# RiceChuan/teku

Measured on AMD Instinct MI355X. Metric: BLS sigs verified/sec (batchVerify), 1-8 GPUs; p50 latency @128-sig batch, higher is better.
Workload: dtype u32 (381-bit Montgomery Fp, 14x29-bit limb products); 1 GPU; config 5 per-GPU shard: randomized batchVerify of 131072 single-signer sets per GPU, RCCL Fp12 partial gather, 1 final exp; sets_per_gpu=131072, parallelism=data-parallel shards, dp1

## Files before the change

__graft_entry__.py:

```python

import os
import subprocess
import sys

ROOT = os.path.dirname(os.path.abspath(__file__))
CSRC = os.path.join(ROOT, "teku_amd", "csrc")
LIBDIR = os.path.join(ROOT, "teku_amd", "lib")
HIPCC = os.environ.get("HIPCC", "/opt/rocm/bin/hipcc")
ARCH = "gfx950"


def _run(cmd):
    print("+", " ".join(cmd), flush=True)
    subprocess.check_call(cmd, cwd=ROOT)


def _stale(out, deps):
    if not os.path.exists(out):
        return True
    t = os.path.getmtime(out)
    return any(os.path.getmtime(d) > t for d in deps)


def _includes(path, seen=None):
    import re

    seen = set() if seen is None else seen
    path = os.path.normpath(path)
    if path in seen or not os.path.exists(path):
        return seen
    seen.add(path)
    for m in re.finditer(r'^\s*#\s*include\s+"([^"]+)"', open(path).read(), re.M):
        _includes(os.path.join(os.path.dirname(path), m.group(1)), seen)
    return seen


def _csrc_deps():
    return [os.path.join(CSRC, f) for f in os.listdir(CSRC) if f.endswith((".h", ".hip"))] + [
        os.path.join(ROOT, "include", "tekubls.h")
    ]


HIP_TUS = ["tb_lib.hip", "tb_kzg.hip", "k_keys.hip", "k_pkindex.hip", "k_sigs.hip", "k_hash.hip", "k_mwave.hip", "k_hwave.hip", "k_hrow.hip", "k_kcoop.hip", "k_lines.hip", "k_pair.hip", "k_each.hip", "k_kzg.hip", "k_w2_hash.hip", "k_w2_sig.hip", "k_w2_pk.hip", "k_hquad.hip", "k_w2_lines.hip", "tb_hostdec.hip"]


def build_hip_lib(force=False, jobs=None, variant=None, defines=(), only=None):
    from concurrent.futures import ThreadPoolExecutor

    os.makedirs(LIBDIR, exist_ok=True)
    objdir = os.path.join(LIBDIR, "obj" if not variant else f"obj_{variant}")
    os.makedirs(objdir, exist_ok=True)
    if variant:
        os.makedirs(os.path.join(LIBDIR, "variants"), exist_ok=True)
    out = os.path.join(LIBDIR, "libtekubls_hip.so" if not variant else os.path.join("variants", f"libtekubls_hip_{variant}.so"))
    deps = _csrc_deps()
    flags = [f"--offload-arch={ARCH}", "-O3", "-std=c++17", "-fPIC"] + [f"-D{d}" for d in defines]

    def compile_tu(tu):
        if variant and only and tu not in only:
            return os.path.join(LIBDIR, "obj", tu.replace(".hip", ".o"))
        obj = os.path.join(objdir, tu.replace(".hip", ".o"))
        if force or _stale(obj, sorted(_includes(os.path.join(CSRC, tu)))):
            _run([HIPCC] + flags + ["-c", os.path.join(CSRC, tu), "-o", obj])
        return obj

    with ThreadPoolExecutor(max_workers=jobs or min(len(HIP_TUS), os.cpu_count() or 4)) as ex:
        objs = list(ex.map(compile_tu, HIP_TUS))
    if force or _stale(out, objs):
        _run([HIPCC, f"--offload-arch={ARCH}", "-shared", "-fPIC"] + objs + ["-o", out])
    return out


def build_test_lib(force=False):
    from concurrent.futures import ThreadPoolExecutor

    d = os.path.join(ROOT, "tests", "native", "_build")
    os.makedirs(d, exist_ok=True)
    out = os.path.join(d, "libtekubls_test.so")
    flags = [f"--offload-arch={ARCH}", "-O3", "-std=c++17", "-fPIC"]

    def compile_tu(name):
        src = os.path.join(ROOT, "tests", "native", name)
        obj = os.path.join(d, name.replace(".hip", ".o"))
        if force or _stale(obj, sorted(_includes(src))):
            _run([HIPCC] + flags + ["-c", src, "-o", obj])
        return obj

    tus = sorted(f for f in os.listdir(os.path.join(ROOT, "tests", "native")) if f.startswith("k_test") and f.endswith(".hip"))
    with ThreadPoolExecutor(max_workers=4) as ex:
        objs = list(ex.map(compile_tu, tus))
    if force or _stale(out, objs):
        _run([HIPCC, f"--offload-arch={ARCH}", "-shared", "-fPIC"] + objs + ["-o", out])
    return out


def build_hostsim(force=False):
    d = os.path.join(ROOT, "tests", "native", "_build")
    os.makedirs(d, exist_ok=True)
    out = os.path.join(d, "libtbhostsim.so")
    src = os.path.join(ROOT, "tests", "native", "hostsim.cpp")
    deps = sorted(_includes(src))
    if force or _stale(out, deps):
        _run(["g++", "-O2", "-std=c++17", "-shared", "-fPIC", src, "-o", out])
    cnt = os.path.join(d, "libtbhostsim_count.so")
    if force or _stale(cnt, deps):
        _run(["g++", "-O1", "-std=c++17", "-DTB_COUNT_MULS", "-shared", "-fPIC", src, "-o", cnt])
    return out


def build_microbench(force=False):
    outs = []
    for name in ("int_rates", "mad_peak", "fp2_rates", "carry_chain"):
        src = os.path.join(ROOT, "tools", "microbench", name + ".hip")
        out = os.path.join(ROOT, "tools", "microbench", name)
        if os.path.exists(src) and (force or _stale(out, sorted(_includes(src)))):
            _run([HIPCC, f"--offload-arch={ARCH}", "-O3", src, "-o", out])
        outs.append(out)
    return outs


def build_oracle(force=False):
    mk = os.path.join(ROOT, "oracle", "c", "Makefile")
    if os.path.exists(mk):
        _run(["make", "-C", os.path.join(ROOT, "oracle", "c"), "-j8"])


# ... 52 lines not shown
```

teku_amd/csrc/k_sigs.hip:

```cpp
#include "tb_kbody.h"

using namespace tb;

extern "C" __global__ void __launch_bounds__(TB_BLOCK, TB_MIN_WAVES)
    k_aggregate_sigs(const uint8_t* __restrict__ sigs, uint32_t K, uint8_t* __restrict__ out, int* __restrict__ status) {
  __shared__ g2j sh[TB_BLOCK];
  __shared__ int bad;
  const int t = threadIdx.x;
  if (t == 0) bad = 0;
  __syncthreads();
  g2j acc = jac_inf<fp2>();
  for (uint32_t i = t; i < K; i += blockDim.x) {
    g2a a;
    bool inf;
    int code = g2_decompress(a, inf, sigs + (size_t)i * 96);
    if (code == TB_SUCCESS && !inf && !g2_in_group(jac_from_aff(a))) code = TB_POINT_NOT_IN_GROUP;
    if (code != TB_SUCCESS)
      atomicCAS(&bad, 0, code);
    else if (!inf)
      acc = jac_add(acc, jac_from_aff(a));
  }
  sh[t] = acc;
  __syncthreads();
  for (int s = TB_BLOCK / 2; s > 0; s >>= 1) {
// ... 43 lines not shown
  uint32_t i = blockIdx.x * blockDim.x + threadIdx.x;
  if (i >= n) return;
  g2a a;
  bool inf;
  int code = g2_decompress(a, inf, sigs + (size_t)i * 96);
  if (code == TB_SUCCESS && !inf && !g2_in_group(jac_from_aff(a))) code = TB_POINT_NOT_IN_GROUP;
  out[i] = (uint32_t)code | (inf ? 0x100u : 0u);
}

#define TB_MSM_W 8
#define TB_MSM_NB 256

extern "C" __global__ void __launch_bounds__(TB_BLOCK, TB_MIN_WAVES) k_g1_comb_init(g1a* __restrict__ comb) {
  const uint32_t t = blockIdx.x * blockDim.x + threadIdx.x;
  if (t >= TB_MSM_W * TB_MSM_NB) return;
  const uint32_t w = t / TB_MSM_NB, d = t % TB_MSM_NB;
  g1a out;
  out.x = fp_zero();
  out.y = fp_zero();
  if (d) {
    g1j g = {fp_from_const(G1_X), fp_from_const(G1_Y), fp_one()};
    for (uint32_t k = 0; k < 8 * w; k++) g = jac_dbl(g);
    (void)jac_to_aff(out, jac_mul_u64(g, d));
  }
  comb[t] = out;
}

extern "C" __global__ void __launch_bounds__(TB_BLOCK, TB_MIN_WAVES)
    k_sig_check(const uint8_t* __restrict__ sigs, uint32_t n, g2a* __restrict__ sig_aff, uint8_t* __restrict__ sig_use,
                uint8_t* __restrict__ sig_code, uint32_t* __restrict__ n_bad, uint32_t skip_mode) {
  const uint32_t i = blockIdx.x * blockDim.x + threadIdx.x;
  if (i >= n) return;
  sig_check_body<false>(i, sigs, sig_aff, sig_use, sig_code, n_bad, skip_mode);
}

extern "C" __global__ void __launch_bounds__(TB_BLOCK, TB_MIN_WAVES)
    k_msm_hist(const uint64_t* __restrict__ rand, uint32_t n, uint32_t* __restrict__ cnt) {
  uint32_t i = blockIdx.x * blockDim.x + threadIdx.x;
  if (i >= n) return;
  const uint64_t r = rand[i];
  for (int w = 0; w < TB_MSM_W; w++) {
    const uint32_t d = (uint32_t)(r >> (8 * w)) & 255u;
    if (d) atomicAdd(&cnt[w * TB_MSM_NB + d], 1u);
  }
}

extern "C" __global__ void __launch_bounds__(256)
    k_msm_scan(const uint32_t* __restrict__ cnt, uint32_t* __restrict__ off, uint32_t* __restrict__ cur) {
  __shared__ uint32_t sh[256];
  const int t = threadIdx.x;
  const int per = TB_MSM_W * TB_MSM_NB / 256;
  uint32_t loc[TB_MSM_W * TB_MSM_NB / 256];
  uint32_t s = 0;
  for (int k = 0; k < per; k++) {
    loc[k] = s;
    s += cnt[t * per + k];
  }
  sh[t] = s;
  __syncthreads();
  for (int d = 1; d < 256; d <<= 1) {
    uint32_t v = t >= d ? sh[t - d] : 0u;
    __syncthreads();
    sh[t] += v;
    __syncthreads();
  }
  const uint32_t base = sh[t] - s;
  for (int k = 0; k < per; k++) {
    off[t * per + k] = base + loc[k];
    cur[t * per + k] = base + loc[k];
  }
  if (t == 255) off[TB_MSM_W * TB_MSM_NB] = sh[t];
}

extern "C" __global__ void __launch_bounds__(TB_BLOCK, TB_MIN_WAVES)
    k_msm_scatter(const uint64_t* __restrict__ rand, uint32_t n, uint32_t* __restrict__ cur, uint32_t* __restrict__ idx) {
  uint32_t i = blockIdx.x * blockDim.x + threadIdx.x;
  if (i >= n) return;
  const uint64_t r = rand[i];
  for (int w = 0; w < TB_MSM_W; w++) {
    const uint32_t d = (uint32_t)(r >> (8 * w)) & 255u;
    if (d) idx[atomicAdd(&cur[w * TB_MSM_NB + d], 1u)] = i;
  }
}

#define TB_MSM_LANES 32u
static_assert(64 % TB_MSM_LANES == 0 && (TB_MSM_W * (TB_MSM_NB - 1)) % (64 / TB_MSM_LANES) == 0, "whole buckets per workgroup");
__device__ TB_INLINE g2j shfl_down_g2j(const g2j& p, int s, int width) {
  g2j r;
  const uint32_t* a = reinterpret_cast<const uint32_t*>(&p);
  uint32_t* o = reinterpret_cast<uint32_t*>(&r);
  TB_UNROLL for (int k = 0; k < (int)(sizeof(g2j) / 4); k++) o[k] = __shfl_down(a[k], s, width);
  return r;
}

extern "C" __global__ void __launch_bounds__(64)
    k_msm_bucket_tree(const g2a* __restrict__ sig_aff, const uint8_t* __restrict__ use, const uint32_t* __restrict__ off,
                      const uint32_t* __restrict__ idx, g2j* __restrict__ bucket) {
  const uint32_t c = threadIdx.x % TB_MSM_LANES;
  const uint32_t q = blockIdx.x * (64 / TB_MSM_LANES) + threadIdx.x / TB_MSM_LANES;
  const uint32_t w = q / (TB_MSM_NB - 1), d = q % (TB_MSM_NB - 1) + 1, b = w * TB_MSM_NB + d;
  const uint32_t lo = off[b], hi = off[b + 1];
  const uint32_t len = hi - lo, chunk = (len + TB_MSM_LANES - 1) / TB_MSM_LANES;
  uint32_t s = lo + c * chunk, e = s + chunk;
  if (e > hi) e = hi;
  g2j acc = jac_inf<fp2>();
  for (uint32_t k = s; k < e; k++) {
    const uint32_t i = idx[k];
    if (use[i]) acc = jac_add_aff(acc, sig_aff[i]);
  }
  for (int sh = TB_MSM_LANES / 2; sh > 0; sh >>= 1) {
    const g2j other = shfl_down_g2j(acc, sh, TB_MSM_LANES);
    if (c < (uint32_t)sh) acc = jac_add(acc, other);
  }
  if (c == 0) bucket[b] = acc;
}

extern "C" __global__ void __launch_bounds__(64)
    k_msm_bitsum_pairs(const g2j* __restrict__ bucket, const g1a* __restrict__ comb, g1a* __restrict__ P, g2a* __restrict__ Q,
                       uint8_t* __restrict__ skip) {
  const uint32_t t = threadIdx.x, w = blockIdx.x / 8, k = blockIdx.x % 8;
  g2j acc = jac_inf<fp2>();
  for (uint32_t r = t; r < 128; r += 64) {
    const uint32_t d = ((r >> k) << (k + 1)) | (1u << k) | (r & ((1u << k) - 1u));
    acc = jac_add(acc, bucket[w * TB_MSM_NB + d]);
  }
  for (int sh = 32; sh > 0; sh >>= 1) {
    const g2j other = shfl_down_g2j(acc, sh, 64);
    if (t < (uint32_t)sh) acc = jac_add(acc, other);
  }
  if (t == 0) {
    g2a a;
    const bool ok = jac_to_aff(a, acc);
    if (!ok) {
      a.x = fp2_zero();
      a.y = fp2_zero();
    }
    g1a c = comb[w * TB_MSM_NB + (1u << k)];
    c.y = fp_neg(c.y);
    P[blockIdx.x] = c;
    Q[blockIdx.x] = a;
    skip[blockIdx.x] = ok ? 0 : 1;
  }
}
```

teku_amd/csrc/tb_lean.h:

```cpp
#pragma once
#include "tb_curve.h"

namespace tb {
namespace lean {

#if defined(__HIP_DEVICE_COMPILE__)
#define TB_LFENCE() __builtin_amdgcn_sched_barrier(0)
#else
#define TB_LFENCE() ((void)0)
#endif

__device__ TB_INLINE fp2 M(const fp2& a, const fp2& b) {
  const fp2 r = fp2_mul(a, b);
  TB_LFENCE();
  return r;
}
__device__ TB_INLINE fp2 S(const fp2& a) {
  const fp2 r = fp2_sqr(a);
  TB_LFENCE();
  return r;
}

__device__ TB_INLINE g2j madd(const g2j& p, const g2a& q) {
  const fp2 Z1Z1 = S(p.z);
  const fp2 H = fp2_sub(M(q.x, Z1Z1), p.x);
  const fp2 r = fp2_dbl(fp2_sub(M(M(q.y, p.z), Z1Z1), p.y));
  const fp2 HH = S(H);
  g2j o;
  o.z = fp2_sub(fp2_sub(S(fp2_add_nr(p.z, H)), Z1Z1), HH);
  const fp2 I = fp2_dbl(fp2_dbl(HH));
  const fp2 J = M(H, I);
  const fp2 V = M(p.x, I);
  o.x = fp2_sub(fp2_sub(S(r), J), fp2_dbl(V));
  o.y = fp2_sub(M(r, fp2_sub(V, o.x)), fp2_dbl(M(p.y, J)));
  return o;
}

template <bool PLUS1 = false>
__device__ TB_INLINE g2j mul_xabs_aff(const g2a& Q, g2a* park) {
  *park = Q;
  asm volatile("" ::: "memory");
  g2j r = jac_from_aff(Q);
  TB_NOUNROLL for (int k = 0; k < 6; k++) {
    const int nd = k == 0 ? 1 : k == 1 ? 2 : k == 2 ? 3 : k == 3 ? 9 : k == 4 ? 32 : 16;
    TB_NOUNROLL for (int i = 0; i < nd; i++) r = jac_dbl_i(r);
    if (PLUS1 || k < 5) r = madd(r, *park);
  }
  return r;
}

struct lds_pt {
  uint4* p;
  __device__ TB_INLINE fp2 ld(int k) const {
    fp2 r;
    TB_UNROLL for (int j = 0; j < 3; j++) {
      const uint4 a = p[(6 * k + j) * TB_BLOCK], b = p[(6 * k + 3 + j) * TB_BLOCK];
      r.c0.l[4 * j] = a.x, r.c0.l[4 * j + 1] = a.y, r.c0.l[4 * j + 2] = a.z, r.c0.l[4 * j + 3] = a.w;
      r.c1.l[4 * j] = b.x, r.c1.l[4 * j + 1] = b.y, r.c1.l[4 * j + 2] = b.z, r.c1.l[4 * j + 3] = b.w;
    }
    return r;
  }
  __device__ TB_INLINE void st(int k, const fp2& v) const {
    TB_UNROLL for (int j = 0; j < 3; j++) {
      p[(6 * k + j) * TB_BLOCK] = make_uint4(v.c0.l[4 * j], v.c0.l[4 * j + 1], v.c0.l[4 * j + 2], v.c0.l[4 * j + 3]);
      p[(6 * k + 3 + j) * TB_BLOCK] = make_uint4(v.c1.l[4 * j], v.c1.l[4 * j + 1], v.c1.l[4 * j + 2], v.c1.l[4 * j + 3]);
    }
    asm volatile("" ::: "memory");
  }
  __device__ TB_INLINE g2j get() const { return {ld(0), ld(1), ld(2)}; }
  __device__ TB_INLINE void put(const g2j& v) const {
    st(0, v.x);
    st(1, v.y);
    st(2, v.z);
  }
};
#define TB_LDS_PT_UINT4 18

__device__ TB_INLINE void dbl_lds(const lds_pt& P) {
  {
    const fp2 y2 = fp2_dbl(P.ld(1));
    P.st(2, M(y2, P.ld(2)));
  }
  const fp2 B = S(P.ld(1));
  const fp2 A = S(P.ld(0));
  const fp2 C = S(B);
  const fp2 D = fp2_dbl(fp2_sub(fp2_sub(S(fp2_add_nr(P.ld(0), B)), A), C));
  const fp2 E = fp2_add_nr(fp2_dbl(A), A);
  const fp2 X3 = fp2_sub(S(E), fp2_dbl(D));
  P.st(0, X3);
  const fp2 C8 = fp2_dbl(fp2_dbl(fp2_dbl(C)));
  P.st(1, fp2_sub(M(E, fp2_sub(D, X3)), C8));
}

__device__ TB_INLINE void madd_lds(const lds_pt& P, const g2a& q) {
  const fp2 Z1Z1 = S(P.ld(2));
  const fp2 H = fp2_sub(M(q.x, Z1Z1), P.ld(0));
  const fp2 r = fp2_dbl(fp2_sub(M(M(q.y, P.ld(2)), Z1Z1), P.ld(1)));
  const fp2 HH = S(H);
  P.st(2, fp2_sub(fp2_sub(S(fp2_add_nr(P.ld(2), H)), Z1Z1), HH));
  const fp2 I = fp2_dbl(fp2_dbl(HH));
  const fp2 J = M(H, I);
  const fp2 V = M(P.ld(0), I);
  const fp2 X3 = fp2_sub(fp2_sub(S(r), J), fp2_dbl(V));
  const fp2 Y3 = fp2_sub(M(r, fp2_sub(V, X3)), fp2_dbl(M(P.ld(1), J)));
  P.st(0, X3);
  P.st(1, Y3);
}

template <bool PLUS1 = false>
__device__ TB_INLINE void mul_xabs_aff_lds(const lds_pt& P, const g2a& Q, g2a* gpark) {
  *gpark = Q;
  asm volatile("" ::: "memory");
  P.put(jac_from_aff(Q));
  TB_NOUNROLL for (int k = 0; k < 6; k++) {
    const int nd = k == 0 ? 1 : k == 1 ? 2 : k == 2 ? 3 : k == 3 ? 9 : k == 4 ? 32 : 16;
    TB_NOUNROLL for (int i = 0; i < nd; i++) dbl_lds(P);
    if (PLUS1 || k < 5) madd_lds(P, *gpark);
  }
}

__device__ TB_INLINE bool to_aff(g2a& o, const g2j& p) {
  if (fp2_is_zero(p.z)) return false;
  const fp2 zi = fp2_inv(p.z);
  const fp2 zi2 = S(zi);
  o.x = M(p.x, zi2);
  o.y = M(M(p.y, zi2), zi);
  return true;
}
__device__ TB_INLINE bool to_aff2(g2a& a, g2a& b, const g2j& p, const g2j& q) {
  const fp2 z = M(p.z, q.z);
  if (fp2_is_zero(z)) return false;
  const fp2 zi = fp2_inv(z);
  const fp2 zp = M(zi, q.z), zq = M(zi, p.z);
  const fp2 zp2 = S(zp), zq2 = S(zq);
  a.x = M(p.x, zp2);
  a.y = M(M(p.y, zp2), zp);
  b.x = M(q.x, zq2);
  b.y = M(M(q.y, zq2), zq);
  return true;
}
__device__ TB_INLINE g2a neg_aff(const g2a& q) { return {q.x, fp2_neg(q.y)}; }
__device__ TB_INLINE g2a psi_aff(const g2a& q) {
  return {M(fp2_conj(q.x), fp2_from_const(PSI_CX)), M(fp2_conj(q.y), fp2_from_const(PSI_CY))};
}

__device__ TB_INLINE bool psi_eq_neg(const g2j& t, const g2a& Q) {
  const fp2 Z2 = S(t.z);
  const bool ex = fp2_is_zero(fp2_sub(M(M(fp2_conj(Q.x), fp2_from_const(PSI_CX)), Z2), t.x));
  const fp2 Z3 = M(Z2, t.z);
  const bool ey = fp2_is_zero(fp2_add(M(M(fp2_conj(Q.y), fp2_from_const(PSI_CY)), Z3), t.y));
  return ex && ey && !fp2_is_zero(t.z);
}

#undef TB_LFENCE
}
}
```

teku_amd/csrc/tb_lib.hip:

```cpp
#include <chrono>
#include <cstdlib>
#include <functional>
#include <cstring>
#include <mutex>
#include <algorithm>
#include <dlfcn.h>
#include <map>
#include <sys/random.h>
#include <rccl/rccl.h>
#include <thread>
#include <type_traits>
#include <vector>

#include "../../include/tekubls.h"
#include "tb_kdecl.h"
#include "tb_hrow.h"
#include "tb_host.h"
#include "tb_pkindex.h"
#include "tb_plan.h"
#include "tb_pack.h"

static_assert(TB_PARTIAL_BYTES == TBLS_PARTIAL_BYTES, "partial record size");
static_assert(tb::plan::LINE_BYTES_PER_PAIR == TB_LINE_BYTES_PER_PAIR, "tb_plan.h: line bytes per pair");
static_assert(tb::plan::HROW_SET_BYTES == sizeof(tb::hrow_set), "tb_plan.h: row-hash workspace per set");
// ... 190 lines not shown
                     comb);
  if (!multi) return;
  (void)hipMemsetAsync(mcnt, 0, 4, s);
  hipLaunchKernelGGL(k_multi_list, g, blk, 0, s, pk_off, n, mlist, mcnt);
  if (multi == 2)
    hipLaunchKernelGGL(k_set_pk_agg_coop, dim3(std::min<uint32_t>(n, 4096u)), dim3(512), 0, s, pk_off, ks.aff, ks.code, rand,
                       (const uint32_t*)mlist, (const uint32_t*)mcnt, P, set_code, n_bad, ks.idx, ks.tab_n, P2, comb, 0u);
  else
    hipLaunchKernelGGL(k_set_pk_wave, dim3(std::min<uint32_t>(n, 4096u)), dim3(64), 0, s, pk_off, ks.aff, ks.code, rand,
                       (const uint32_t*)mlist, (const uint32_t*)mcnt, P, set_code, n_bad, ks.idx, ks.tab_n);
}

#define TB_CM_WORDS (TBLS_COMMITTEE_MAX / 32)
#define TB_CM_OFF_BAD ((size_t)TBLS_COMMITTEE_MAX * 4)
#define TB_CM_OFF_VALID (TB_CM_OFF_BAD + 256)
#define TB_CM_OFF_SUM (TB_CM_OFF_VALID + 256)
#define TB_CM_OFF_CODE (TB_CM_OFF_SUM + 256)
#define TB_CM_STRIDE (TB_CM_OFF_CODE + 256)
struct bits_src {
  const uint32_t *members, *bad;
  const g1a* sum;
  uint32_t size, sum_ok, stride_w;
};
inline bits_src committee_src(const dev_ctx& c, uint32_t slot) {
  const uint8_t* m = c.cmt.as<const uint8_t>((size_t)slot * TB_CM_STRIDE);
  return {(const uint32_t*)m, (const uint32_t*)(m + TB_CM_OFF_BAD), (const g1a*)(m + TB_CM_OFF_SUM), c.cm_size[slot], c.cm_sum_ok[slot],
          bits_stride_w(c.cm_size[slot])};
}

void launch_set_pk_bits(hipStream_t s, uint32_t n, const key_src& ks, const bits_src& cm, const uint64_t* rand, g1a* P, uint8_t* set_code,
                        uint32_t* n_bad, g1a* P2, const g1a* comb, uint32_t unit_r) {
  if (!n) return;
  hipLaunchKernelGGL(k_set_pk_bits_coop, dim3(std::min<uint32_t>(n, 4096u)), dim3(512), 0, s, ks.idx, cm.stride_w, cm.members, cm.size, cm.bad,
                     cm.sum, cm.sum_ok, ks.aff, ks.code, ks.tab_n, rand, n, P, set_code, n_bad, P2, comb, unit_r);
}

#define TB_PKX_BLOCK 256u

inline uint32_t pkx_align(const void* p) {
  const uintptr_t a = (uintptr_t)p;
  return !(a & 15u) ? 16u : !(a & 3u) ? 4u : 1u;
}

inline bool pk_lookup_on(const dev_ctx& c) { return c.tab_n && c.pkx_cap; }

int pk_lookup_reserve(dev_ctx& c, uint32_t K, hipStream_t s) {
  const size_t need = ((size_t)K + 1) * 4;
  if (!pk_lookup_on(c) || need <= c.pkx_miss.cap) return TBLS_SUCCESS;
  HIPCHK(hipStreamSynchronize(s));
  return c.pkx_miss.ensure(need) ? TBLS_DEVICE_ERROR : TBLS_SUCCESS;
}

int launch_pk_lookup(dev_ctx& c, hipStream_t s, const uint8_t* pks, uint32_t K, g1a* pk_aff, uint8_t* pk_code) {
  uint32_t* miss = c.pkx_miss.as<uint32_t>();
  HIPCHK(hipMemsetAsync(miss, 0, 4, s));
  hipLaunchKernelGGL(k_pk_lookup, dim3((K + TB_PKX_BLOCK - 1) / TB_PKX_BLOCK), dim3(TB_PKX_BLOCK), 0, s, pks, K, pkx_align(pks),
                     c.pkx_slots.as<const uint32_t>(), c.pkx_cap - 1u, c.pkx_seed, c.tab_keys.as<const uint32_t>(), c.tab_aff.as<const g1a>(),
                     c.tab_code.as<const uint8_t>(), pk_aff, pk_code, miss, c.pkx_stat.as<unsigned long long>());
  return TBLS_SUCCESS;
}
int launch_byte_keys(dev_ctx& c, hipStream_t s, const uint8_t* pks, uint32_t K, g1a* pk_aff, uint8_t* pk_code, bool looked_up = false) {
  if (!K) return TBLS_SUCCESS;
  const dim3 blk(TB_BLOCK), g((K + TB_BLOCK - 1) / TB_BLOCK);
  if (!pk_lookup_on(c)) {
    hipLaunchKernelGGL(k_pk_decompress, g, blk, 0, s, pks, K, pk_aff, pk_code);
    return TBLS_SUCCESS;
  }
  if (!looked_up)
    if (const int rc = launch_pk_lookup(c, s, pks, K, pk_aff, pk_code)) return rc;
  hipLaunchKernelGGL(k_pk_decompress_list, g, blk, 0, s, pks, c.pkx_miss.as<const uint32_t>(), pk_aff, pk_code);
  return TBLS_SUCCESS;
}

struct partial_run {
  dev_ctx& c;
  const tbls_dev_batch& b;
  const partial_opts& o;
  const batch_plan& bp;
  const ws_ptrs& W;
  const key_src& keys;
  hipStream_t s, sa, sb, sh;
  bool late_join;
  bool pre_lookup;
  const uint32_t n = b.n;
  const dim3 blk = dim3(TB_BLOCK), g = dim3((b.n + TB_BLOCK - 1) / TB_BLOCK);
  g1a* sig_P() const { return bp.pp.msm ? nullptr : W.P + n; }

#define TB_EV(i, st) \
  if (o.ev) HIPCHK(hipEventRecord(o.ev[i], st))

  int sig_chain() const {
    const pair_plan& pp = bp.pp;
    if (pp.msm) {
      HIPCHK(hipMemsetAsync(W.msm_cnt, 0, TB_MSM_BUCKETS * 4, sb));
      hipLaunchKernelGGL(k_msm_hist, g, blk, 0, sb, b.rand, n, W.msm_cnt);
      hipLaunchKernelGGL(k_msm_scan, dim3(1), dim3(256), 0, sb, (const uint32_t*)W.msm_cnt, W.msm_off, W.msm_cur);
      hipLaunchKernelGGL(k_msm_scatter, g, blk, 0, sb, b.rand, n, W.msm_cur, W.msm_idx);
    }
    TB_EV(4, sb);
    if (n) {
      const auto check = bp.w2 ? k_sig_check_w2 : k_sig_check;
      if (bp.sig == sig_kind::msm)
        hipLaunchKernelGGL(check, g, blk, 0, sb, b.sigs, n, W.sig_aff, W.sig_use, W.sig_code, W.n_bad, 0u);
      else if (bp.sig == sig_kind::coop)
        hipLaunchKernelGGL(k_sig_check_coop, dim3((n + 3) / 4), dim3(64), 0, sb, b.sigs, n, W.Q + n, W.skip + n, W.sig_code, W.n_bad);
      else
        hipLaunchKernelGGL(check, g, blk, 0, sb, b.sigs, n, W.Q + n, W.skip + n, W.sig_code, W.n_bad, 1u);
    }
    TB_EV(5, sb);
    if (late_join) HIPCHK(hipEventRecord(c.e_sig, sb));
    TB_EV(8, sb);
    if (pp.msm) {
      hipLaunchKernelGGL(k_msm_bucket_tree, dim3(TB_MSM_TREE_WG), dim3(64), 0, sb, (const g2a*)W.sig_aff, (const uint8_t*)W.sig_use,
                         (const uint32_t*)W.msm_off, (const uint32_t*)W.msm_idx, W.msm_sum);
      hipLaunchKernelGGL(k_msm_bitsum_pairs, dim3(TB_MSM_XPAIRS), dim3(64), 0, sb, (const g2j*)W.msm_sum, c.comb.as<const g1a>(), W.P + n,
                         W.Q + n, W.skip + n);
      if (pp.n_xwave)
        hipLaunchKernelGGL(k_miller_wave, dim3(pp.n_xwave), dim3(64), 0, sb, (const g1a*)W.P + n, (const g2a*)W.Q + n, (const uint8_t*)W.skip + n,
                           (const uint8_t*)W.set_code + n, (const uint8_t*)W.sig_code + n, pp.n_xwave, W.f + pp.n_f_main());
    }
    TB_EV(9, sb);
    return TBLS_SUCCESS;
  }

  int key_chain() const {
    const g1a* comb = c.comb.as<const g1a>();
    if (!pre_lookup) TB_EV(0, sa);
    if (bp.key == key_kind::bits) {
      TB_EV(1, sa);
      TB_EV(2, sa);
      launch_set_pk_bits(sa, n, keys, *o.cm, b.rand, W.P, W.set_code, W.n_bad, sig_P(), comb, 0u);
    } else if (bp.key == key_kind::keys_coop) {
      const bool tab = keys.idx != nullptr;
      hipLaunchKernelGGL(k_keys_coop, dim3((n + 3) / 4), dim3(128), 0, sa, tab ? nullptr : b.pks, b.pk_off, tab ? keys.aff : nullptr,
                         tab ? keys.code : nullptr, keys.idx, keys.tab_n, b.rand, n, W.P, sig_P(), W.set_code, W.n_bad, comb);
      TB_EV(1, sa);
      TB_EV(2, sa);
    } else {
      if (const int rc = launch_byte_keys(c, sa, b.pks, bp.n_keys, W.pk_aff, W.pk_code, pre_lookup)) return rc;
      TB_EV(1, sa);
      TB_EV(2, sa);
      launch_set_pk(sa, n, bp.w2, bp.multi, b.pk_off, keys, b.rand, W.P, W.set_code, W.n_bad, W.mlist, W.mcnt, sig_P(), comb);
    }
    TB_EV(3, sa);
    return TBLS_SUCCESS;
  }

  int hash_chain() const {
    g2a* Q = W.Q;
    uint8_t* skip = W.skip;
    TB_EV(6, sh);
    switch (bp.hash) {
      case hash_kind::none:
        break;
      case hash_kind::coop:
        hipLaunchKernelGGL(k_set_hash_coop, dim3(n), dim3(256), 0, sh, b.msgs, b.msg_off, o.dst, o.dlen, n, Q, skip, (const uint64_t*)nullptr);
        break;
      case hash_kind::wave:
        hipLaunchKernelGGL(k_set_hash_wave, dim3(n), dim3(128), 0, sh, b.msgs, b.msg_off, o.dst, o.dlen, n, Q, skip);
        break;
      case hash_kind::row: {
        hrow_set* H = W.hrow;
        hipLaunchKernelGGL(k_hrow_field, g, blk, 0, sh, b.msgs, b.msg_off, o.dst, o.dlen, n, H);
        hipLaunchKernelGGL(k_hrow_sswu, dim3((2 * n + 3) / 4), dim3(64), 0, sh, n, H);
        hipLaunchKernelGGL(k_hrow_iso, g, blk, 0, sh, n, H);
        hipLaunchKernelGGL(k_hrow_cof, dim3((n + 3) / 4), dim3(64), 0, sh, n, (const hrow_set*)H, Q, skip, 0);
        hipLaunchKernelGGL(k_hrow_fix, g, blk, 0, sh, n, (const hrow_set*)H, Q, skip);
        break;
      }
      case hash_kind::quad:
        hipLaunchKernelGGL(k_set_hash_quad, dim3((4 * n + TB_BLOCK - 1) / TB_BLOCK), blk, 0, sh, b.msgs, b.msg_off, o.dst, o.dlen, n, Q, skip);
        break;
      case hash_kind::duo:
        hipLaunchKernelGGL(k_set_hash_duo, dim3((2 * n + TB_BLOCK - 1) / TB_BLOCK), blk, 0, sh, b.msgs, b.msg_off, o.dst, o.dlen, n, Q, skip);
        break;
      case hash_kind::w2:
        hipLaunchKernelGGL(k_set_hash_w2, g, blk, 0, sh, b.msgs, b.msg_off, o.dst, o.dlen, n, Q, skip, (g2a*)W.lines);
        break;
      case hash_kind::lane:
        hipLaunchKernelGGL(k_set_hash, g, blk, 0, sh, b.msgs, b.msg_off, o.dst, o.dlen, n, Q, skip);
        break;
    }
    if (bp.hash == hash_kind::quad || bp.hash == hash_kind::duo || bp.hash == hash_kind::w2)
      hipLaunchKernelGGL(k_set_hash_fix, g, blk, 0, sh, b.msgs, b.msg_off, o.dst, o.dlen, n, Q, skip);
    TB_EV(7, sh);
    return TBLS_SUCCESS;
  }

  int miller() const {
    const pair_plan& pp = bp.pp;
    const uint32_t np = pp.n_pairs;
    const g1a* P = W.P;
    const g2a* Q = W.Q;
    const uint8_t *skip = W.skip, *ca = W.set_code, *cb = W.sig_code;
    TB_EV(10, s);
    if (!np) return TBLS_SUCCESS;
    if (pp.wave) {
      hipLaunchKernelGGL(k_miller_wave, dim3(np), dim3(64), 0, s, P, Q, skip, ca, cb, np, W.f);
      return TBLS_SUCCESS;
    }
    const uint4* lines = W.lines;
    const auto line_kernel = bp.line_group == 4 ? k_miller_lines_quad : bp.line_group == 2 ? k_miller_lines_duo : k_miller_lines_w2;
    for (uint32_t lo = 0; lo < pp.n_main; lo += TB_LINE_CHUNK) {
      const uint32_t m = std::min(TB_LINE_CHUNK, pp.n_main - lo), mt = (m + pp.per - 1) / pp.per;
      hipLaunchKernelGGL(line_kernel, dim3((bp.line_group * m + TB_BLOCK - 1) / TB_BLOCK), blk, 0, s, P + lo, Q + lo, skip + lo, ca + lo, cb + lo, m,
                         W.lines);
      if (o.settle) continue;
      if (late_join && lo == 0) HIPCHK(hipStreamWaitEvent(s, c.e_join[1], 0));
      if (pp.seg()) {
        const uint32_t g_pad = (mt + TB_BLOCK - 1) / TB_BLOCK * TB_BLOCK;
        hipLaunchKernelGGL(k_miller_accs_lds, dim3(pp.nseg * g_pad / TB_BLOCK), blk, 0, s, lines, skip + lo, ca + lo, cb + lo, m, pp.per, pp.nseg,
                           g_pad, W.f + lo / pp.per, pp.n_groups());
      } else {
        hipLaunchKernelGGL(pp.per == 2 ? k_miller_acc2 : k_miller_acc1, dim3((mt + TB_BLOCK - 1) / TB_BLOCK), blk, 0, s, lines, skip + lo, ca + lo,
                           cb + lo, m, W.f + lo / pp.per);
      }
    }
    return TBLS_SUCCESS;
  }

  int product_tree(void* partial_out) const {
    TB_EV(12, s);
    if (bp.pp.n_f() == 0) {
      HIPCHK(hipMemsetAsync(W.f, 0, sizeof(fp12), s));
      hipLaunchKernelGGL(k_fp12_one, dim3(1), dim3(64), 0, s, W.f);
    }
    const fp12* src = W.f;
    for (int i = 0; i < bp.n_levels; i++) {
      const prod_level& l = bp.levels[i];
      fp12* out = l.dst == prod_dst::partial ? (fp12*)partial_out : l.dst == prod_dst::segv ? W.segv : l.dst == prod_dst::fpart2 ? W.fpart2 : W.fpart;
      if (l.seg)
        hipLaunchKernelGGL(k_fp12_prod_wave_seg, dim3(l.n_out, bp.pp.nseg), dim3(64), 0, s, src, l.n_in, l.n_in_last, bp.pp.nseg, l.in_stride,
                           l.chunk, out, l.out_stride);
      else
        hipLaunchKernelGGL(k_fp12_prod_wave, dim3(l.n_out), dim3(64), 0, s, src, l.n_in, l.chunk, out);
      src = out;
    }
    if (bp.combine)
      hipLaunchKernelGGL(k_fp12_seg_combine_coop, dim3(1), dim3(TB_CFE_THREADS), 0, s, (const fp12*)W.segv, bp.pp.nseg, 0u, (fp12*)partial_out);
    TB_EV(13, s);
    return TBLS_SUCCESS;
  }
};

int launch_partial(dev_ctx& c, const tbls_dev_batch& b, hipStream_t s, void* partial_out, ws_layout& L, const partial_opts& o) {
  const batch_plan bp(b.n, b.n_keys, o.cm ? key_source::bits : o.key_idx ? key_source::table : key_source::bytes, o.settle);
  L = ws_layout(bp);
  tb::stat_add(tb::TB_STAT_PARTIALS);
  HIPCHK(ws_acquire(c, s));
  if (L.total > c.ws.cap) {
    HIPCHK(hipStreamSynchronize(s));
    if (c.ws.ensure(L.total)) return TBLS_DEVICE_ERROR;
  }
  if (bp.key == key_kind::decompress)
    if (const int rc = pk_lookup_reserve(c, bp.n_keys, s)) return rc;
  const ws_ptrs W(L, c.ws.as<uint8_t>());
  const key_src keys = o.key_idx ? table_keys(c, o.key_idx) : own_keys(W.pk_aff, W.pk_code);
  const bool late_join = bp.late_join && !o.serial;
  const bool pre_lookup = bp.key == key_kind::decompress && bp.n_keys && pk_lookup_on(c) && !o.serial;
  const partial_run run{c, b, o, bp, W, keys, s, o.serial ? s : c.aux[0], o.serial ? s : c.aux[1], o.serial ? s : c.aux[2], late_join, pre_lookup};
  HIPCHK(hipMemsetAsync(W.set_code, 0, 2 * align_up(bp.pp.n_pairs), s));
  HIPCHK(hipMemsetAsync(W.n_bad, 0, 4, s));
  if (run.pre_lookup) {
    if (o.ev) HIPCHK(hipEventRecord(o.ev[0], s));
    if (const int rc = launch_pk_lookup(c, s, b.pks, bp.n_keys, W.pk_aff, W.pk_code)) return rc;
  }
  if (!o.serial) {
    HIPCHK(hipEventRecord(c.e_fork, s));
    HIPCHK(hipStreamWaitEvent(run.sa, c.e_fork, 0));
    HIPCHK(hipStreamWaitEvent(run.sb, c.e_fork, 0));
    HIPCHK(hipStreamWaitEvent(run.sh, c.e_fork, 0));
  }
  if (const int rc = run.sig_chain()) return rc;
  HIPCHK(hipEventRecord(c.e_join[1], run.sb));
  if (const int rc = run.key_chain()) return rc;
  HIPCHK(hipEventRecord(c.e_join[0], run.sa));
  if (late_join && bp.sig_first) HIPCHK(hipStreamWaitEvent(run.sh, c.e_sig, 0));
  if (const int rc = run.hash_chain()) return rc;
  if (!o.serial) {
    HIPCHK(hipEventRecord(c.e_join[2], run.sh));
    HIPCHK(hipStreamWaitEvent(s, c.e_join[2], 0));
  }
  HIPCHK(hipStreamWaitEvent(s, c.e_join[0], 0));
  if (!late_join)
    HIPCHK(hipStreamWaitEvent(s, c.e_join[1], 0));
  else
    HIPCHK(hipStreamWaitEvent(s, c.e_sig, 0));
  if (const int rc = run.miller()) return rc;
  if (late_join) HIPCHK(hipStreamWaitEvent(s, c.e_join[1], 0));
  if (o.settle) {
    HIPCHK(hipGetLastError());
    HIPCHK(ws_release(c, s));
    return TBLS_SUCCESS;
  }
  TB_EV(11, s);
  if (const int rc = run.product_tree(partial_out)) return rc;
  HIPCHK(hipMemcpyAsync((uint8_t*)partial_out + sizeof(fp12), W.n_bad, 4, hipMemcpyDeviceToDevice, s));
  HIPCHK(hipGetLastError());
  HIPCHK(ws_release(c, s));
  return TBLS_SUCCESS;
}
#undef TB_EV

int launch_final(dev_ctx& c, const void* recs, uint32_t g, hipStream_t s, int* result_host) {
  if (c.fin.ensure(256)) return TBLS_DEVICE_ERROR;
  int* res = c.fin.as<int>();
  tb::stat_add(tb::TB_STAT_FINALS);
  tb_launch_final_recs((const uint8_t*)recs, g, s, res);
  HIPCHK(hipGetLastError());
  if (c.hout.ensure(16)) return TBLS_DEVICE_ERROR;
  HIPCHK(hipMemcpyAsync(c.hout.p, res, 4, hipMemcpyDeviceToHost, s));
  HIPCHK(hipStreamSynchronize(s));
  *result_host = *(int*)c.hout.p;
  return TBLS_SUCCESS;
}

int ensure_init() {
  std::lock_guard<std::mutex> lk(g_mu);
  if (g_inited) return g_ctx.empty() ? TBLS_DEVICE_ERROR : TBLS_SUCCESS;
  return TBLS_DEVICE_ERROR;
}

dev_ctx* ctx_for(int d) {
  if (d < 0 || d >= (int)g_ctx.size()) return nullptr;
  return g_ctx[d];
}

template <class SET>
int check_keys(const dev_ctx* c, const SET* sets, size_t lo, size_t hi) {
  if constexpr (std::is_same<SET, tbls_set_idx>::value) {
    if (!c->tab_n) return TBLS_BAD_ARGUMENT;
    for (size_t i = lo; i < hi; i++)
      for (uint32_t k = 0; k < sets[i].n_pks; k++)
        if (sets[i].key_idx[k] >= c->tab_n) return TBLS_BAD_ARGUMENT;
  } else if constexpr (std::is_same<SET, set_bits_i>::value) {
    if (!c->tab_n) return TBLS_BAD_ARGUMENT;
    for (size_t i = lo; i < hi; i++)
      if (sets[i].slot >= TBLS_COMMITTEE_SLOTS || sets[i].slot != sets[lo].slot || !sets[i].size ||
          sets[i].size != c->cm_size[sets[i].slot] || sets[i].n_pks != bits_stride_w(sets[i].size))
        return TBLS_BAD_ARGUMENT;
  }
  return TBLS_SUCCESS;
}

const uint8_t ETH2_DST[] = "BLS_SIG_BLS12381G2_XMD:SHA-256_SSWU_RO_POP_";

template <class SET>
int shard_launch(dev_ctx* c, const SET* sets, size_t lo, size_t hi, const uint64_t* rand, const uint8_t* dst, uint32_t dlen,
                 uint8_t** dpart, ws_layout& L, uint32_t* n_out, bool settle = false) {
// ... 1172 lines not shown
```

teku_amd/csrc/tb_plan.h:

```cpp
#pragma once
#include <algorithm>
#include <cmath>
#include <cstdint>
#include <cstdio>
#include <cstdlib>
#include <vector>

#include "tb_curve.h"

namespace tb {
namespace plan {

inline size_t align_up(size_t x, size_t a = 256) { return (x + a - 1) / a * a; }

constexpr size_t LINE_BYTES_PER_PAIR = 68u * 288u;
constexpr size_t HROW_SET_BYTES = 864;

#define TB_SHARD_MIN 32768u
#define TB_SHARD_KNEE 4096u
#define TB_PROD_CHUNK 16u
#define TB_MSM_MIN 20480u
#define TB_HASH_WAVE_MAX 512u
#define TB_MSM_BUCKETS 2048u
#define TB_MSM_NSUM 2040u
#define TB_MSM_TREE_WG (TB_MSM_NSUM / 2u)
#define TB_MSM_XPAIRS 64u
#define TB_LINE_CHUNK 262144u
#define TB_MILLER_PER2_MIN 131072u
#define TB_MILLER_WAVE_MAX 2048u
#define TB_ACC_FULL 65536u
#define TB_ACC_PER_MAX 16
#define TB_ACC_NSEG_MAX 16
#define TB_HASH_ROW_MAX 1024u
#define TB_HASH_QUAD_MAX 8192u
#define TB_HASH_DUO_MAX 32768u
#define TB_GROUP_LANES 65536u
#ifndef TB_PROD_SMALL_MAX
#define TB_PROD_SMALL_MAX 4096u
#endif
#define TB_W2_MIN 32768u
#define TB_SETTLE_FAN 16u
#define TB_SETTLE_MAX (TB_LINE_CHUNK / 2u)

struct plan_env {
  uint32_t msm_min = TB_MSM_MIN;
  uint32_t miller_wave_max = TB_MILLER_WAVE_MAX;
  int acc_per = -1, acc_seg = -1;
  uint32_t row_max = TB_HASH_ROW_MAX, quad_max = TB_HASH_QUAD_MAX, duo_max = TB_HASH_DUO_MAX;
  bool w2 = true;
  bool coop = true;
  uint32_t shard_min = TB_SHARD_MIN, shard_knee = TB_SHARD_KNEE;

  void parse_msm_min(const char* v) {
    if (v) msm_min = (uint32_t)atoi(v);
  }
  void parse_miller_wave_max(const char* v) {
    if (v) miller_wave_max = (uint32_t)atoi(v);
  }
  void parse_acc_plan(const char* v) {
    acc_per = acc_seg = -1;
    if (!v) return;
    if (v[0] == '0' && v[1] == 0) {
      acc_per = acc_seg = 0;
      return;
    }
    int p = 0, g = 0;
    if (sscanf(v, "%d,%d", &p, &g) == 2 && p >= 1 && p <= 32 && (p & (p - 1)) == 0 && g >= 1 && g <= TB_ACC_NSEG_MAX) {
      acc_per = p;
      acc_seg = g;
    }
  }
  void parse_hash_plan(const char* v) {
    unsigned r, q, d;
    if (v && sscanf(v, "%u,%u,%u", &r, &q, &d) == 3) {
      row_max = r;
      quad_max = q;
      duo_max = d;
    }
  }
  void parse_w2(const char* v) { w2 = !(v && v[0] == '0'); }
  void parse_coop(const char* v) { coop = !(v && v[0] == '0'); }
  void parse_shard_min(const char* v) {
    if (!v) return;
    unsigned a = 0, b = 0;
    const int k = sscanf(v, "%u,%u", &a, &b);
    if (k >= 1) shard_min = a;
    shard_knee = k == 2 ? b : std::min(shard_min, (uint32_t)TB_SHARD_KNEE);
  }

  static plan_env from_environment() {
    plan_env e;
    e.parse_msm_min(getenv("TBLS_MSM_MIN"));
    e.parse_miller_wave_max(getenv("TBLS_MILLER_WAVE_MAX"));
    e.parse_acc_plan(getenv("TBLS_ACC_PLAN"));
    e.parse_hash_plan(getenv("TBLS_HASH_PLAN"));
    e.parse_w2(getenv("TBLS_W2"));
    e.parse_coop(getenv("TBLS_COOP"));
    e.parse_shard_min(getenv("TBLS_SHARD_MIN"));
    return e;
  }
  static const plan_env& get() {
    static const plan_env v = from_environment();
    return v;
  }
};

template <class KEYS>
int place_plan(size_t n, const KEYS& keys, int D, int n_gpus, const int* load, uint32_t rr, uint32_t smin, uint32_t knee, int* dev,
               size_t* cut) {
// ... 256 lines not shown
```

Measured before the change: 3.779 million sigs/s.

## Move MSM bucket accumulation to LDS-resident lean points with wider lanes and pre-sort

```diff
diff --git a/__graft_entry__.py b/__graft_entry__.py
--- a/__graft_entry__.py
+++ b/__graft_entry__.py
@@ -41,7 +41,7 @@
     ]
 
 
-HIP_TUS = ["tb_lib.hip", "tb_kzg.hip", "k_keys.hip", "k_pkindex.hip", "k_sigs.hip", "k_hash.hip", "k_mwave.hip", "k_hwave.hip", "k_hrow.hip", "k_kcoop.hip", "k_lines.hip", "k_pair.hip", "k_each.hip", "k_kzg.hip", "k_w2_hash.hip", "k_w2_sig.hip", "k_w2_pk.hip", "k_hquad.hip", "k_w2_lines.hip", "tb_hostdec.hip"]
+HIP_TUS = ["tb_lib.hip", "tb_kzg.hip", "k_keys.hip", "k_pkindex.hip", "k_sigs.hip", "k_hash.hip", "k_mwave.hip", "k_hwave.hip", "k_hrow.hip", "k_kcoop.hip", "k_lines.hip", "k_pair.hip", "k_each.hip", "k_kzg.hip", "k_w2_hash.hip", "k_w2_sig.hip", "k_w2_msm.hip", "k_w2_pk.hip", "k_hquad.hip", "k_w2_lines.hip", "tb_hostdec.hip"]
 
 
 def build_hip_lib(force=False, jobs=None, variant=None, defines=(), only=None):
diff --git a/teku_amd/csrc/k_sigs.hip b/teku_amd/csrc/k_sigs.hip
--- a/teku_amd/csrc/k_sigs.hip
+++ b/teku_amd/csrc/k_sigs.hip
@@ -149,63 +149,3 @@
     if (d) idx[atomicAdd(&cur[w * TB_MSM_NB + d], 1u)] = i;
   }
 }
-
-#define TB_MSM_LANES 32u
-static_assert(64 % TB_MSM_LANES == 0 && (TB_MSM_W * (TB_MSM_NB - 1)) % (64 / TB_MSM_LANES) == 0, "whole buckets per workgroup");
-__device__ TB_INLINE g2j shfl_down_g2j(const g2j& p, int s, int width) {
-  g2j r;
-  const uint32_t* a = reinterpret_cast<const uint32_t*>(&p);
-  uint32_t* o = reinterpret_cast<uint32_t*>(&r);
-  TB_UNROLL for (int k = 0; k < (int)(sizeof(g2j) / 4); k++) o[k] = __shfl_down(a[k], s, width);
-  return r;
-}
-
-extern "C" __global__ void __launch_bounds__(64)
-    k_msm_bucket_tree(const g2a* __restrict__ sig_aff, const uint8_t* __restrict__ use, const uint32_t* __restrict__ off,
-                      const uint32_t* __restrict__ idx, g2j* __restrict__ bucket) {
-  const uint32_t c = threadIdx.x % TB_MSM_LANES;
-  const uint32_t q = blockIdx.x * (64 / TB_MSM_LANES) + threadIdx.x / TB_MSM_LANES;
-  const uint32_t w = q / (TB_MSM_NB - 1), d = q % (TB_MSM_NB - 1) + 1, b = w * TB_MSM_NB + d;
-  const uint32_t lo = off[b], hi = off[b + 1];
-  const uint32_t len = hi - lo, chunk = (len + TB_MSM_LANES - 1) / TB_MSM_LANES;
-  uint32_t s = lo + c * chunk, e = s + chunk;
-  if (e > hi) e = hi;
-  g2j acc = jac_inf<fp2>();
-  for (uint32_t k = s; k < e; k++) {
-    const uint32_t i = idx[k];
-    if (use[i]) acc = jac_add_aff(acc, sig_aff[i]);
-  }
-  for (int sh = TB_MSM_LANES / 2; sh > 0; sh >>= 1) {
-    const g2j other = shfl_down_g2j(acc, sh, TB_MSM_LANES);
-    if (c < (uint32_t)sh) acc = jac_add(acc, other);
-  }
-  if (c == 0) bucket[b] = acc;
-}
-
-extern "C" __global__ void __launch_bounds__(64)
-    k_msm_bitsum_pairs(const g2j* __restrict__ bucket, const g1a* __restrict__ comb, g1a* __restrict__ P, g2a* __restrict__ Q,
-                       uint8_t* __restrict__ skip) {
-  const uint32_t t = threadIdx.x, w = blockIdx.x / 8, k = blockIdx.x % 8;
-  g2j acc = jac_inf<fp2>();
-  for (uint32_t r = t; r < 128; r += 64) {
-    const uint32_t d = ((r >> k) << (k + 1)) | (1u << k) | (r & ((1u << k) - 1u));
-    acc = jac_add(acc, bucket[w * TB_MSM_NB + d]);
-  }
-  for (int sh = 32; sh > 0; sh >>= 1) {
-    const g2j other = shfl_down_g2j(acc, sh, 64);
-    if (t < (uint32_t)sh) acc = jac_add(acc, other);
-  }
-  if (t == 0) {
-    g2a a;
-    const bool ok = jac_to_aff(a, acc);
-    if (!ok) {
-      a.x = fp2_zero();
-      a.y = fp2_zero();
-    }
-    g1a c = comb[w * TB_MSM_NB + (1u << k)];
-    c.y = fp_neg(c.y);
-    P[blockIdx.x] = c;
-    Q[blockIdx.x] = a;
-    skip[blockIdx.x] = ok ? 0 : 1;
-  }
-}
diff --git a/teku_amd/csrc/k_w2_msm.hip b/teku_amd/csrc/k_w2_msm.hip
--- /dev/null
+++ b/teku_amd/csrc/k_w2_msm.hip
@@ -0,0 +1,138 @@
+#include "tb_kbody.h"
+#include "tb_lean.h"
+#include "tb_msm.h"
+
+using namespace tb;
+
+#define TB_MSM_W 8
+#define TB_MSM_NB 256
+static_assert(TB_MSM_WG == 256 && TB_MSM_WG % TB_MSM_LANES == 0 && TB_MSM_LANES >= 4, "whole buckets per workgroup; 128 and 64 lanes on the tree's first levels");
+static_assert(TB_MSM_W * (TB_MSM_NB - 1) == TB_MSM_NSUM && TB_MSM_TREE_WG * (TB_MSM_WG / TB_MSM_LANES) == TB_MSM_NSUM, "whole workgroups over the buckets");
+static_assert(TB_MSM_XPAIRS == TB_MSM_W * 8, "one workgroup per (window, bit)");
+static_assert(TB_BLOCK == 64, "lds_pt's layout is one wave wide");
+
+__device__ TB_INLINE lean::lds_pt msm_slot(uint4* sh, uint32_t s) { return {sh + (s >> 6) * (TB_LDS_PT_UINT4 * TB_BLOCK) + (s & 63u)}; }
+
+__device__ TB_INLINE g2j msm_from_aff(const g2a& q) {
+  fp2 one = fp2_one();
+  TB_UNROLL for (int j = 0; j < 12; j++) asm volatile("" : "+v"(one.c0.l[j]));
+  return {q.x, q.y, one};
+}
+
+__device__ TB_INLINE void msm_tree_add(uint4* sh, uint32_t* inf, uint32_t a, uint32_t b) {
+  if (inf[b]) return;
+  const lean::lds_pt A = msm_slot(sh, a), B = msm_slot(sh, b);
+  if (inf[a]) {
+    A.put(B.get());
+    inf[a] = 0;
+    return;
+  }
+  const int c = lean::add_lds_chk(A, B);
+  if (c == 1) {
+    A.put(B.get());
+    lean::dbl_lds(A);
+  } else if (c == 2) {
+    inf[a] = 1;
+  }
+}
+
+template <uint32_t L>
+__device__ TB_INLINE bool msm_lds_tree(uint4* sh, uint32_t* inf, uint32_t t) {
+  constexpr uint32_t G = TB_MSM_WG / L;
+  __syncthreads();
+  if (t < G * (L / 2)) msm_tree_add(sh, inf, (t / (L / 2)) * L + t % (L / 2), (t / (L / 2)) * L + t % (L / 2) + L / 2);
+  __syncthreads();
+  if (t >= 64) return false;
+  TB_NOUNROLL for (uint32_t h = L / 4; h > 0; h >>= 1) {
+    if (t < G * h) msm_tree_add(sh, inf, (t / h) * L + t % h, (t / h) * L + t % h + h);
+    __builtin_amdgcn_fence(__ATOMIC_ACQ_REL, "workgroup");
+    __builtin_amdgcn_wave_barrier();
+  }
+  return true;
+}
+
+extern "C" __global__ void __launch_bounds__(TB_MSM_WG, 2)
+    k_msm_bucket_tree(const g2a* __restrict__ sig_aff, const uint8_t* __restrict__ use, const uint32_t* __restrict__ off,
+                    const uint32_t* __restrict__ idx, g2j* __restrict__ bucket) {
+  __shared__ uint4 Psh[TB_LDS_PT_UINT4 * TB_MSM_WG];
+  __shared__ uint32_t Inf[TB_MSM_WG];
+  constexpr uint32_t G = TB_MSM_WG / TB_MSM_LANES;
+  const uint32_t t = threadIdx.x, c = t % TB_MSM_LANES;
+  {
+    const uint32_t q = blockIdx.x * G + t / TB_MSM_LANES;
+    const uint32_t b = (q / (TB_MSM_NB - 1)) * TB_MSM_NB + q % (TB_MSM_NB - 1) + 1;
+    const uint32_t lo = off[b], hi = off[b + 1];
+    const uint32_t chunk = (hi - lo + TB_MSM_LANES - 1) / TB_MSM_LANES;
+    uint32_t s = lo + c * chunk, e = s + chunk;
+    if (s > hi) s = hi;
+    if (e > hi) e = hi;
+    const lean::lds_pt P = msm_slot(Psh, t);
+    bool inf = true;
+    TB_NOUNROLL for (uint32_t k = s; k < e; k++) {
+      const uint32_t i = idx[k];
+      if (!use[i]) continue;
+      if (inf) {
+        P.put(msm_from_aff(sig_aff[i]));
+        inf = false;
+        continue;
+      }
+      const int r = lean::madd_lds_chk(P, sig_aff[i]);
+      if (r == 1)
+        lean::dbl_lds(P);
+      else if (r == 2)
+        inf = true;
+    }
+    Inf[t] = inf ? 1u : 0u;
+  }
+  if (!msm_lds_tree<TB_MSM_LANES>(Psh, Inf, t) || t >= G) return;
+  const uint32_t q = blockIdx.x * G + t;
+  const uint32_t b = (q / (TB_MSM_NB - 1)) * TB_MSM_NB + q % (TB_MSM_NB - 1) + 1;
+  bucket[b] = Inf[t * TB_MSM_LANES] ? jac_inf<fp2>() : msm_slot(Psh, t * TB_MSM_LANES).get();
+}
+
+extern "C" __global__ void __launch_bounds__(TB_BLOCK, 2)
+    k_msm_bitsum_pairs(const g2j* __restrict__ bucket, const g1a* __restrict__ comb, g1a* __restrict__ P, g2a* __restrict__ Q,
+                       uint8_t* __restrict__ skip) {
+  __shared__ uint4 Psh[TB_LDS_PT_UINT4 * TB_BLOCK];
+  __shared__ uint32_t Inf[TB_BLOCK];
+  const uint32_t t = threadIdx.x, w = blockIdx.x / 8, k = blockIdx.x % 8;
+  {
+    const lean::lds_pt A = msm_slot(Psh, t);
+    bool inf = true;
+    TB_NOUNROLL for (uint32_t r = t; r < 128; r += 64) {
+      const uint32_t d = ((r >> k) << (k + 1)) | (1u << k) | (r & ((1u << k) - 1u));
+      const lean::glb_pt B{bucket + w * TB_MSM_NB + d};
+      if (fp2_is_zero(B.ld(2))) continue;
+      if (inf) {
+        A.put(B.get());
+        inf = false;
+        continue;
+      }
+      const int c = lean::add_lds_chk(A, B);
+      if (c == 1) {
+        A.put(B.get());
+        lean::dbl_lds(A);
+      } else if (c == 2) {
+        inf = true;
+      }
+    }
+    Inf[t] = inf ? 1u : 0u;
+  }
+  TB_NOUNROLL for (uint32_t h = 32; h > 0; h >>= 1) {
+    __builtin_amdgcn_fence(__ATOMIC_ACQ_REL, "workgroup");
+    __builtin_amdgcn_wave_barrier();
+    if (t < h) msm_tree_add(Psh, Inf, t, t + h);
+  }
+  if (t) return;
+  g2a a;
+  const bool ok = !Inf[0] && lean::to_aff(a, msm_slot(Psh, 0).get());
+  if (!ok) {
+    a.x = fp2_zero();
+    a.y = fp2_zero();
+  }
+  g1a c = comb[w * TB_MSM_NB + (1u << k)];
+  c.y = fp_neg(c.y);
+  P[blockIdx.x] = c;
+  Q[blockIdx.x] = a;
+  skip[blockIdx.x] = ok ? 0 : 1;
+}
diff --git a/teku_amd/csrc/tb_lean.h b/teku_amd/csrc/tb_lean.h
--- a/teku_amd/csrc/tb_lean.h
+++ b/teku_amd/csrc/tb_lean.h
@@ -105,6 +105,54 @@
   const fp2 Y3 = fp2_sub(M(r, fp2_sub(V, X3)), fp2_dbl(M(P.ld(1), J)));
   P.st(0, X3);
   P.st(1, Y3);
+}
+
+__device__ TB_INLINE int madd_lds_chk(const lds_pt& P, const g2a& q) {
+  const fp2 Z1Z1 = S(P.ld(2));
+  const fp2 H = fp2_sub(M(q.x, Z1Z1), P.ld(0));
+  const fp2 r = fp2_dbl(fp2_sub(M(M(q.y, P.ld(2)), Z1Z1), P.ld(1)));
+  if (fp2_is_zero(H)) return fp2_is_zero(r) ? 1 : 2;
+  const fp2 HH = S(H);
+  P.st(2, fp2_sub(fp2_sub(S(fp2_add_nr(P.ld(2), H)), Z1Z1), HH));
+  const fp2 I = fp2_dbl(fp2_dbl(HH));
+  const fp2 J = M(H, I);
+  const fp2 V = M(P.ld(0), I);
+  const fp2 X3 = fp2_sub(fp2_sub(S(r), J), fp2_dbl(V));
+  const fp2 Y3 = fp2_sub(M(r, fp2_sub(V, X3)), fp2_dbl(M(P.ld(1), J)));
+  P.st(0, X3);
+  P.st(1, Y3);
+  return 0;
+}
+
+struct glb_pt {
+  const g2j* p;
+  __device__ TB_INLINE fp2 ld(int k) const {
+    asm volatile("" ::: "memory");
+    return k == 0 ? p->x : k == 1 ? p->y : p->z;
+  }
+  __device__ TB_INLINE g2j get() const { return *p; }
+};
+
+template <class PB>
+__device__ TB_INLINE int add_lds_chk(const lds_pt& A, const PB& B) {
+  {
+    const fp2 Z2Z2 = S(B.ld(2));
+    A.st(0, M(A.ld(0), Z2Z2));
+    A.st(1, M(M(A.ld(1), B.ld(2)), Z2Z2));
+  }
+  const fp2 Z1Z1 = S(A.ld(2));
+  const fp2 H = fp2_sub(M(B.ld(0), Z1Z1), A.ld(0));
+  const fp2 r = fp2_dbl(fp2_sub(M(M(B.ld(1), A.ld(2)), Z1Z1), A.ld(1)));
+  if (fp2_is_zero(H)) return fp2_is_zero(r) ? 1 : 2;
+  A.st(2, M(fp2_dbl(M(A.ld(2), B.ld(2))), H));
+  const fp2 I = S(fp2_dbl(H));
+  const fp2 J = M(H, I);
+  const fp2 V = M(A.ld(0), I);
+  const fp2 X3 = fp2_sub(fp2_sub(S(r), J), fp2_dbl(V));
+  const fp2 Y3 = fp2_sub(M(r, fp2_sub(V, X3)), fp2_dbl(M(A.ld(1), J)));
+  A.st(0, X3);
+  A.st(1, Y3);
+  return 0;
 }
 
 template <bool PLUS1 = false>
diff --git a/teku_amd/csrc/tb_lib.hip b/teku_amd/csrc/tb_lib.hip
--- a/teku_amd/csrc/tb_lib.hip
+++ b/teku_amd/csrc/tb_lib.hip
@@ -296,6 +296,7 @@
   hipStream_t s, sa, sb, sh;
   bool late_join;
   bool pre_lookup;
+  bool pre_sort;
   const uint32_t n = b.n;
   const dim3 blk = dim3(TB_BLOCK), g = dim3((b.n + TB_BLOCK - 1) / TB_BLOCK);
   g1a* sig_P() const { return bp.pp.msm ? nullptr : W.P + n; }
@@ -303,14 +304,18 @@
 #define TB_EV(i, st) \
   if (o.ev) HIPCHK(hipEventRecord(o.ev[i], st))
 
+  int msm_sort(hipStream_t st) const {
+    HIPCHK(hipMemsetAsync(W.msm_cnt, 0, TB_MSM_BUCKETS * 4, st));
+    hipLaunchKernelGGL(k_msm_hist, g, blk, 0, st, b.rand, n, W.msm_cnt);
+    hipLaunchKernelGGL(k_msm_scan, dim3(1), dim3(256), 0, st, (const uint32_t*)W.msm_cnt, W.msm_off, W.msm_cur);
+    hipLaunchKernelGGL(k_msm_scatter, g, blk, 0, st, b.rand, n, W.msm_cur, W.msm_idx);
+    return TBLS_SUCCESS;
+  }
+
   int sig_chain() const {
     const pair_plan& pp = bp.pp;
-    if (pp.msm) {
-      HIPCHK(hipMemsetAsync(W.msm_cnt, 0, TB_MSM_BUCKETS * 4, sb));
-      hipLaunchKernelGGL(k_msm_hist, g, blk, 0, sb, b.rand, n, W.msm_cnt);
-      hipLaunchKernelGGL(k_msm_scan, dim3(1), dim3(256), 0, sb, (const uint32_t*)W.msm_cnt, W.msm_off, W.msm_cur);
-      hipLaunchKernelGGL(k_msm_scatter, g, blk, 0, sb, b.rand, n, W.msm_cur, W.msm_idx);
-    }
+    if (pp.msm && !pre_sort)
+      if (const int rc = msm_sort(sb)) return rc;
     TB_EV(4, sb);
     if (n) {
       const auto check = bp.w2 ? k_sig_check_w2 : k_sig_check;
@@ -325,7 +330,7 @@
     if (late_join) HIPCHK(hipEventRecord(c.e_sig, sb));
     TB_EV(8, sb);
     if (pp.msm) {
-      hipLaunchKernelGGL(k_msm_bucket_tree, dim3(TB_MSM_TREE_WG), dim3(64), 0, sb, (const g2a*)W.sig_aff, (const uint8_t*)W.sig_use,
+      hipLaunchKernelGGL(k_msm_bucket_tree, dim3(TB_MSM_TREE_WG), dim3(TB_MSM_WG), 0, sb, (const g2a*)W.sig_aff, (const uint8_t*)W.sig_use,
                          (const uint32_t*)W.msm_off, (const uint32_t*)W.msm_idx, W.msm_sum);
       hipLaunchKernelGGL(k_msm_bitsum_pairs, dim3(TB_MSM_XPAIRS), dim3(64), 0, sb, (const g2j*)W.msm_sum, c.comb.as<const g1a>(), W.P + n,
                          W.Q + n, W.skip + n);
@@ -472,13 +477,15 @@
   const key_src keys = o.key_idx ? table_keys(c, o.key_idx) : own_keys(W.pk_aff, W.pk_code);
   const bool late_join = bp.late_join && !o.serial;
   const bool pre_lookup = bp.key == key_kind::decompress && bp.n_keys && pk_lookup_on(c) && !o.serial;
-  const partial_run run{c, b, o, bp, W, keys, s, o.serial ? s : c.aux[0], o.serial ? s : c.aux[1], o.serial ? s : c.aux[2], late_join, pre_lookup};
+  const partial_run run{c, b, o, bp, W, keys, s, o.serial ? s : c.aux[0], o.serial ? s : c.aux[1], o.serial ? s : c.aux[2], late_join, pre_lookup, bp.pp.msm && !o.serial};
   HIPCHK(hipMemsetAsync(W.set_code, 0, 2 * align_up(bp.pp.n_pairs), s));
   HIPCHK(hipMemsetAsync(W.n_bad, 0, 4, s));
   if (run.pre_lookup) {
     if (o.ev) HIPCHK(hipEventRecord(o.ev[0], s));
     if (const int rc = launch_pk_lookup(c, s, b.pks, bp.n_keys, W.pk_aff, W.pk_code)) return rc;
   }
+  if (run.pre_sort)
+    if (const int rc = run.msm_sort(s)) return rc;
   if (!o.serial) {
     HIPCHK(hipEventRecord(c.e_fork, s));
     HIPCHK(hipStreamWaitEvent(run.sa, c.e_fork, 0));
diff --git a/teku_amd/csrc/tb_msm.h b/teku_amd/csrc/tb_msm.h
--- /dev/null
+++ b/teku_amd/csrc/tb_msm.h
@@ -0,0 +1,8 @@
+#pragma once
+#define TB_MSM_NSUM 2040u
+#define TB_MSM_XPAIRS 64u
+#define TB_MSM_WG 256u
+#ifndef TB_MSM_LANES
+#define TB_MSM_LANES 64u
+#endif
+#define TB_MSM_TREE_WG (TB_MSM_NSUM / (TB_MSM_WG / TB_MSM_LANES))
diff --git a/teku_amd/csrc/tb_plan.h b/teku_amd/csrc/tb_plan.h
--- a/teku_amd/csrc/tb_plan.h
+++ b/teku_amd/csrc/tb_plan.h
@@ -7,6 +7,7 @@
 #include <vector>
 
 #include "tb_curve.h"
+#include "tb_msm.h"
 
 namespace tb {
 namespace plan {
@@ -22,9 +23,6 @@
 #define TB_MSM_MIN 20480u
 #define TB_HASH_WAVE_MAX 512u
 #define TB_MSM_BUCKETS 2048u
-#define TB_MSM_NSUM 2040u
-#define TB_MSM_TREE_WG (TB_MSM_NSUM / 2u)
-#define TB_MSM_XPAIRS 64u
 #define TB_LINE_CHUNK 262144u
 #define TB_MILLER_PER2_MIN 131072u
 #define TB_MILLER_WAVE_MAX 2048u
```

New measurement: 3.425 million sigs/s. 9.4% lower.
